# pythoncrazy/jimm

Measured on NVIDIA H100. Metric: images/sec, higher is better.
Workload: dtype f16

## Files before the change

### jimm_b200/csrc/common.cuh

```cuda
#pragma once

#include <cuda.h>
#include <cuda_bf16.h>
#include <cuda_fp16.h>
#include <cuda_fp8.h>
#include <cuda_runtime.h>
#include <stdint.h>

#include <atomic>
#include <mutex>
#include <string>

namespace jimm {

void set_last_error(const char* fmt, ...);

#define JIMM_CUDA_CHECK(expr)                                                                   \
  do {                                                                                          \
    cudaError_t _e = (expr);                                                                    \
    if (_e != cudaSuccess) {                                                                    \
      ::jimm::set_last_error("%s:%d: %s -> %s", __FILE__, __LINE__, #expr, cudaGetErrorString(_e)); \
      return -2;                                                                                \
    }                                                                                           \
  } while (0)
// ... 80 lines not shown
      : "=r"(pred));
  return pred != 0;
}

__device__ __forceinline__ void mbar_init(uint64_t* bar, uint32_t count) {
  asm volatile("mbarrier.init.shared::cta.b64 [%0], %1;" ::"r"(smem_u32(bar)), "r"(count));
}
__device__ __forceinline__ void fence_barrier_init() {
  asm volatile("fence.mbarrier_init.release.cluster;" ::: "memory");
}
__device__ __forceinline__ void fence_proxy_async_smem() {
  asm volatile("fence.proxy.async.shared::cta;" ::: "memory");
}
__device__ __forceinline__ void mbar_arrive(uint64_t* bar) {
  asm volatile("mbarrier.arrive.shared::cta.b64 _, [%0];" ::"r"(smem_u32(bar)) : "memory");
}
__device__ __forceinline__ void mbar_arrive_expect_tx(uint64_t* bar, uint32_t bytes) {
  asm volatile("mbarrier.arrive.expect_tx.shared::cta.b64 _, [%0], %1;" ::"r"(smem_u32(bar)), "r"(bytes) : "memory");
}
__device__ __forceinline__ void mbar_wait(uint64_t* bar, uint32_t parity) {
  asm volatile(
      "{\n\t.reg .pred P1;\n\t"
      "WAIT_LOOP:\n\t"
      "mbarrier.try_wait.parity.shared::cta.b64 P1, [%0], %1;\n\t"
      "@P1 bra DONE;\n\t"
      "bra WAIT_LOOP;\n\t"
      "DONE:\n\t}" ::"r"(smem_u32(bar)),
      "r"(parity)
      : "memory");
}

__device__ __forceinline__ bool mbar_test_wait(uint64_t* bar, uint32_t parity) {
  uint32_t ok;
  asm volatile(
      "{\n\t.reg .pred P1;\n\t"
      "mbarrier.test_wait.parity.shared::cta.b64 P1, [%1], %2;\n\t"
      "selp.u32 %0, 1, 0, P1;\n\t}"
      : "=r"(ok)
      : "r"(smem_u32(bar)), "r"(parity)
      : "memory");
  return ok != 0;
}

__device__ __forceinline__ void tma_prefetch_desc(const CUtensorMap* m) {
  asm volatile("prefetch.tensormap [%0];" ::"l"(reinterpret_cast<uint64_t>(m)) : "memory");
}
__device__ __forceinline__ void tma_load_2d(void* smem_dst, const CUtensorMap* m, uint64_t* bar, int c0, int c1) {
  asm volatile(
      "cp.async.bulk.tensor.2d.shared::cluster.global.mbarrier::complete_tx::bytes [%0], [%1, {%3, %4}], [%2];" ::"r"(
          smem_u32(smem_dst)),
      "l"(reinterpret_cast<uint64_t>(m)), "r"(smem_u32(bar)), "r"(c0), "r"(c1)
      : "memory");
}

__device__ __forceinline__ void tma_store_2d(const CUtensorMap* m, uint32_t smem_src, int c0, int c1) {
  asm volatile("cp.async.bulk.tensor.2d.global.shared::cta.bulk_group [%0, {%2, %3}], [%1];" ::"l"(reinterpret_cast<uint64_t>(m)),
               "r"(smem_src), "r"(c0), "r"(c1)
               : "memory");
}
__device__ __forceinline__ void tma_reduce_add_2d(const CUtensorMap* m, uint32_t smem_src, int c0, int c1) {
  asm volatile("cp.reduce.async.bulk.tensor.2d.global.shared::cta.add.tile.bulk_group [%0, {%2, %3}], [%1];" ::"l"(
                   reinterpret_cast<uint64_t>(m)),
               "r"(smem_src), "r"(c0), "r"(c1)
               : "memory");
}
__device__ __forceinline__ void tma_store_3d(const CUtensorMap* m, uint32_t smem_src, int c0, int c1, int c2) {
  asm volatile("cp.async.bulk.tensor.3d.global.shared::cta.bulk_group [%0, {%2, %3, %4}], [%1];" ::"l"(reinterpret_cast<uint64_t>(m)),
               "r"(smem_src), "r"(c0), "r"(c1), "r"(c2)
               : "memory");
}
__device__ __forceinline__ void tma_reduce_add_3d(const CUtensorMap* m, uint32_t smem_src, int c0, int c1, int c2) {
  asm volatile("cp.reduce.async.bulk.tensor.3d.global.shared::cta.add.tile.bulk_group [%0, {%2, %3, %4}], [%1];" ::"l"(
                   reinterpret_cast<uint64_t>(m)),
               "r"(smem_src), "r"(c0), "r"(c1), "r"(c2)
               : "memory");
}
__device__ __forceinline__ void tma_store_commit() { asm volatile("cp.async.bulk.commit_group;" ::: "memory"); }
__device__ __forceinline__ void tma_store_wait_read() { asm volatile("cp.async.bulk.wait_group.read 0;" ::: "memory"); }
__device__ __forceinline__ void tma_store_wait_read1() { asm volatile("cp.async.bulk.wait_group.read 1;" ::: "memory"); }
__device__ __forceinline__ void tma_store_wait_all() { asm volatile("cp.async.bulk.wait_group 0;" ::: "memory"); }

__device__ __forceinline__ uint32_t cluster_ctarank() {
  uint32_t r;
  asm volatile("mov.u32 %0, %%cluster_ctarank;" : "=r"(r));
  return r;
}
__device__ __forceinline__ void cluster_sync_all() {
  asm volatile("barrier.cluster.arrive.release.aligned;\n\tbarrier.cluster.wait.acquire.aligned;" ::: "memory");
}
__device__ __forceinline__ uint32_t mapa_shared(uint32_t local_smem_addr, uint32_t rank) {
  uint32_t r;
  asm volatile("mapa.shared::cluster.u32 %0, %1, %2;" : "=r"(r) : "r"(local_smem_addr), "r"(rank));
  return r;
}
__device__ __forceinline__ void mbar_arrive_cluster(uint32_t cluster_addr) {
  asm volatile("mbarrier.arrive.release.cluster.shared::cluster.b64 _, [%0];" ::"r"(cluster_addr) : "memory");
}
__device__ __forceinline__ uint64_t make_wgmma_desc_sw128(uint32_t smem_addr) {
  uint64_t d = 0;
  d |= static_cast<uint64_t>((smem_addr & 0x3FFFFu) >> 4);
  d |= static_cast<uint64_t>(1) << 16;
  d |= static_cast<uint64_t>(1024 >> 4) << 32;
  d |= static_cast<uint64_t>(1) << 62;
  return d;
}
template <int SW>
__device__ __forceinline__ uint64_t make_wgmma_desc(uint32_t smem_addr, uint32_t lbo) {
  static_assert(SW == 128 || SW == 64 || SW == 32, "swizzle width");
  constexpr uint64_t layout = SW == 128 ? 1 : SW == 64 ? 2 : 3;
  uint64_t d = 0;
  d |= static_cast<uint64_t>((smem_addr & 0x3FFFFu) >> 4);
  d |= static_cast<uint64_t>((lbo >> 4) & 0x3FFFu) << 16;
  d |= static_cast<uint64_t>(8 * SW >> 4) << 32;
  d |= layout << 62;
  return d;
}
__device__ __forceinline__ void wgmma_fence() { asm volatile("wgmma.fence.sync.aligned;" ::: "memory"); }
__device__ __forceinline__ void wgmma_commit() { asm volatile("wgmma.commit_group.sync.aligned;" ::: "memory"); }
template <int N>
__device__ __forceinline__ void wgmma_wait() { asm volatile("wgmma.wait_group.sync.aligned %0;" ::"n"(N) : "memory"); }
template <int R>
__device__ __forceinline__ void wgmma_fence_operands(float (&d)[R]) {
#pragma unroll
  for (int i = 0; i < R; ++i) asm volatile("" : "+f"(d[i])::"memory");
}

#define JIMM_WGMMA_D128                                                                                                                    \
  "{%0, %1, %2, %3, %4, %5, %6, %7, %8, %9, %10, %11, %12, %13, %14, %15, %16, %17, %18, %19, %20, %21, %22, %23, %24, %25, %26, %27, "     \
  "%28, %29, %30, %31, %32, %33, %34, %35, %36, %37, %38, %39, %40, %41, %42, %43, %44, %45, %46, %47, %48, %49, %50, %51, %52, %53, %54, " \
  "%55, %56, %57, %58, %59, %60, %61, %62, %63, %64, %65, %66, %67, %68, %69, %70, %71, %72, %73, %74, %75, %76, %77, %78, %79, %80, %81, " \
  "%82, %83, %84, %85, %86, %87, %88, %89, %90, %91, %92, %93, %94, %95, %96, %97, %98, %99, %100, %101, %102, %103, %104, %105, %106, "   \
  "%107, %108, %109, %110, %111, %112, %113, %114, %115, %116, %117, %118, %119, %120, %121, %122, %123, %124, %125, %126, %127}"
#define JIMM_WGMMA_D8(i) "+f"(d[i]), "+f"(d[i + 1]), "+f"(d[i + 2]), "+f"(d[i + 3]), "+f"(d[i + 4]), "+f"(d[i + 5]), "+f"(d[i + 6]), "+f"(d[i + 7])
#define JIMM_WGMMA_D128_OPERANDS                                                                                                 \
  JIMM_WGMMA_D8(0), JIMM_WGMMA_D8(8), JIMM_WGMMA_D8(16), JIMM_WGMMA_D8(24), JIMM_WGMMA_D8(32), JIMM_WGMMA_D8(40), JIMM_WGMMA_D8(48), \
      JIMM_WGMMA_D8(56), JIMM_WGMMA_D8(64), JIMM_WGMMA_D8(72), JIMM_WGMMA_D8(80), JIMM_WGMMA_D8(88), JIMM_WGMMA_D8(96),             \
      JIMM_WGMMA_D8(104), JIMM_WGMMA_D8(112), JIMM_WGMMA_D8(120)
template <int KIND>
__device__ __forceinline__ void wgmma_m64n256_ss(float (&d)[128], uint64_t adesc, uint64_t bdesc, uint32_t accumulate) {
  if constexpr (KIND == 0) {
    asm volatile("{\n\t.reg .pred p;\n\tsetp.ne.b32 p, %130, 0;\n\t"
                 "wgmma.mma_async.sync.aligned.m64n256k16.f32.f16.f16 " JIMM_WGMMA_D128 ", %128, %129, p, 1, 1, 0, 0;\n\t}"
                 : JIMM_WGMMA_D128_OPERANDS
                 : "l"(adesc), "l"(bdesc), "r"(accumulate));
  } else if constexpr (KIND == 1) {
    asm volatile("{\n\t.reg .pred p;\n\tsetp.ne.b32 p, %130, 0;\n\t"
                 "wgmma.mma_async.sync.aligned.m64n256k16.f32.bf16.bf16 " JIMM_WGMMA_D128 ", %128, %129, p, 1, 1, 0, 0;\n\t}"
                 : JIMM_WGMMA_D128_OPERANDS
                 : "l"(adesc), "l"(bdesc), "r"(accumulate));
// ... 260 lines not shown
```

### jimm_b200/csrc/gemm.cu

```cuda
#include "gemm.cuh"

#include <stdarg.h>
#include <stdio.h>
#include <stdlib.h>
#include <string.h>

#include <type_traits>

#include "common.cuh"

namespace jimm {

static constexpr int BM = GEMM_TILE_M;
static constexpr int BN = GEMM_TILE_N;
static_assert(BM == 128 && BN == 256, "the warp roles and the wgmma shape below are written for 128 x 256 tiles");
static constexpr int STAGES = 4;
static constexpr int A_STAGE_BYTES = BM * 128;
static constexpr int B_STAGE_BYTES = BN * 128;
static constexpr int STAGE_BYTES = A_STAGE_BYTES + B_STAGE_BYTES;
static constexpr int EPI_WARPS = 8;
static constexpr int EPI_BOX_ROWS = 16;
static constexpr int EPI_BUF_BYTES = EPI_BOX_ROWS * 128;
static constexpr int EPI_BUFS = 2;
static constexpr int EPI_STAGE_BYTES = EPI_WARPS * EPI_BUFS * EPI_BUF_BYTES;
// ... 288 lines not shown
    float sa = 1.f;
    if constexpr (SCALED) sa = __ldg(epi.a_scale + row);
#pragma unroll
    for (int j = 0; j < NC / 8; ++j) {
#pragma unroll
      for (int q = 0; q < 2; ++q) {
        const int col = n_tile0 + 8 * j + 2 * t + q;
        if (col < epi.N) {
          float v = acc[4 * j + 2 * h + q];
          if constexpr (SCALED) v *= sa * __ldg(epi.b_scale + col);
          if (epi.bias) v += __ldg(epi.bias + col);
          v = apply_act(v, epi.act);
          if (epi.rowadd) v += __ldg(epi.rowadd + static_cast<size_t>(add_row) * epi.N + col);
          if (epi.residual) v += epi.residual[static_cast<size_t>(out_row) * epi.ldr + col];
          store1(epi, out_row, col, v);
        }
      }
    }
  }
}


template <typename T, int OUT, int ACT>
__global__ void __launch_bounds__(NUM_THREADS, 1)
gemm_wgmma_kernel(const __grid_constant__ CUtensorMap map_a, const __grid_constant__ CUtensorMap map_b,
                  const __grid_constant__ CUtensorMap map_c, const EpiDev epi, int K) {
  constexpr bool SCALED = kScaled<T>;
  constexpr int BK = 128 / sizeof(T);
  constexpr int UK = 32 / sizeof(T);
  constexpr int TM = tile_rows(Traits<T>::DTYPE);
  constexpr int STAGE_TX = TM * 128 + B_STAGE_BYTES;
  constexpr int WG_DM = SCALED ? 0 : 64;
  constexpr int WG_DN = SCALED ? 128 : 0;
  constexpr int NC = BN - WG_DN;
  constexpr bool FUSE_LN = OUT == OUT_F32_ADD && ACT == ACT_FUSE_LN;
  constexpr int EPI_ACT = ACT == ACT_FUSE_LN ? static_cast<int>(ACT_NONE) : ACT;
  constexpr int PRODUCER_REGS = FUSE_LN ? 152 : 40;
  constexpr int CONSUMER_REGS = FUSE_LN ? 176 : 232;
  static_assert(128 * PRODUCER_REGS + 256 * CONSUMER_REGS <= NUM_THREADS * KERNEL_REGS, "register split exceeds the CTA's allocation");

  extern __shared__ uint8_t smem_raw[];
  uint8_t* smem = reinterpret_cast<uint8_t*>((reinterpret_cast<uintptr_t>(smem_raw) + 1023) & ~static_cast<uintptr_t>(1023));
  uint8_t* smem_a = smem;
  uint8_t* smem_b = smem + STAGES * A_STAGE_BYTES;
  uint8_t* epi_stage = smem + STAGES * STAGE_BYTES;
  LnQueue* lnq = reinterpret_cast<LnQueue*>(epi_stage + EPI_STAGE_BYTES);
  uint64_t* full_bar = reinterpret_cast<uint64_t*>(lnq + 1);
  uint64_t* empty_bar = full_bar + STAGES;

  const int warp_idx = threadIdx.x >> 5;
  const int lane = threadIdx.x & 31;
  const int M = epi.M, N = epi.N;
  const int m_tiles = (M + TM - 1) / TM, n_tiles = (N + BN - 1) / BN;
  const int num_tiles = m_tiles * n_tiles;
  const int num_kb = (K + BK - 1) / BK;

  pdl_launch_dependents();
  if (warp_idx == 0 && lane == 0) {
    tma_prefetch_desc(&map_a);
    tma_prefetch_desc(&map_b);
    if constexpr (OUT != OUT_GENERIC) tma_prefetch_desc(&map_c);
    for (int s = 0; s < STAGES; ++s) {
      mbar_init(&full_bar[s], 1);
      mbar_init(&empty_bar[s], EPI_WARPS);
    }
    fence_barrier_init();
  }
  if constexpr (FUSE_LN) {
    if (warp_idx == 1) {
      for (int i = lane; i < LNQ; i += 32) lnq->slot[i] = -1;
      if (lane == 0) lnq->head = lnq->tail = lnq->done = 0;
    }
  }
  __syncthreads();
  pdl_wait();

  if (warp_idx < 4) {
    setmaxnreg<KERNEL_REGS, PRODUCER_REGS>();
    if (warp_idx == 0) {
      if (lane == 0) {
        int stage = 0;
        uint32_t phase = 0;
        for (int tile = blockIdx.x; tile < num_tiles; tile += gridDim.x) {
          const int tv = epi.reverse ? num_tiles - 1 - tile : tile;
          const int m_blk = tv / n_tiles, n_blk = tv - m_blk * n_tiles;
          for (int kb = 0; kb < num_kb; ++kb) {
            mbar_wait(&empty_bar[stage], phase ^ 1);
            mbar_arrive_expect_tx(&full_bar[stage], STAGE_TX);
            tma_load_2d(smem_a + stage * A_STAGE_BYTES, &map_a, &full_bar[stage], kb * BK, m_blk * TM);
            tma_load_2d(smem_b + stage * B_STAGE_BYTES, &map_b, &full_bar[stage], kb * BK, n_blk * BN);
            if (++stage == STAGES) { stage = 0; phase ^= 1; }
          }
        }
      }
    } else if constexpr (FUSE_LN) {
      ln_worker<T>(epi, lnq, lane);
    }
  } else {
    setmaxnreg<KERNEL_REGS, CONSUMER_REGS>();
    const int wg = (warp_idx - 4) >> 2;
    const int wq = warp_idx & 3;
    uint8_t* tbuf0 = epi_stage + (warp_idx - 4) * EPI_BUFS * EPI_BUF_BYTES;
    int stage = 0;
    uint32_t phase = 0, box_count = 0;
    int ln_rg = -1, ln_cols = 0;
    float acc[NC / 2];
    for (int tile = blockIdx.x; tile < num_tiles; tile += gridDim.x) {
      const int tv = epi.reverse ? num_tiles - 1 - tile : tile;
      const int m_blk = tv / n_tiles, n_blk = tv - m_blk * n_tiles;
      int prev = -1;
      if constexpr (SCALED) {
#pragma unroll
        for (int i = 0; i < NC / 2; ++i) acc[i] = 0.f;
      }
      for (int kb = 0; kb < num_kb; ++kb) {
        mbar_wait(&full_bar[stage], phase);
        const uint64_t adesc = make_wgmma_desc_sw128(smem_u32(smem_a + stage * A_STAGE_BYTES + wg * WG_DM * 128));
        const uint64_t bdesc = make_wgmma_desc_sw128(smem_u32(smem_b + stage * B_STAGE_BYTES + wg * WG_DN * 128));
        if constexpr (SCALED) {
          float slab[NC / 2];
          wgmma_fence_operands(slab);
          wgmma_fence();
#pragma unroll
          for (int k = 0; k < BK / UK; ++k)
            wgmma_m64n128k32_e4m3_ss(slab, adesc + static_cast<uint64_t>(2 * k), bdesc + static_cast<uint64_t>(2 * k), k != 0 ? 1u : 0u);
          wgmma_commit();
          wgmma_wait<0>();
          wgmma_fence_operands(slab);
          if (lane == 0) mbar_arrive(&empty_bar[stage]);
#pragma unroll
          for (int i = 0; i < NC / 2; ++i) acc[i] += slab[i];
        } else {
          wgmma_fence_operands(acc);
          wgmma_fence();
#pragma unroll
          for (int k = 0; k < BK / UK; ++k)
            wgmma_m64n256_ss<Traits<T>::KIND>(acc, adesc + static_cast<uint64_t>(2 * k), bdesc + static_cast<uint64_t>(2 * k), (kb | k) != 0 ? 1u : 0u);
          wgmma_commit();
          wgmma_fence_operands(acc);
          if (prev >= 0) {
            wgmma_wait<1>();
            if (lane == 0) mbar_arrive(&empty_bar[prev]);
          }
          prev = stage;
        }
        if (++stage == STAGES) { stage = 0; phase ^= 1; }
      }
      if constexpr (!SCALED) {
        wgmma_wait<0>();
        wgmma_fence_operands(acc);
        if (lane == 0) mbar_arrive(&empty_bar[prev]);
      }

      const int row_base = m_blk * TM + wg * WG_DM + wq * 16;
      const int n_tile0 = n_blk * BN + wg * WG_DN;
      if constexpr (OUT == OUT_GENERIC) {
        epilogue_generic<SCALED, NC>(epi, acc, lane, row_base, n_tile0);
      } else {
        if (row_base < M && (WG_DN == 0 || n_tile0 < N))
          epilogue_tma<OUT, EPI_ACT, SCALED, NC>(&map_c, epi, acc, tbuf0, lane, row_base, n_tile0, box_count);
        if constexpr (FUSE_LN) {
          if (lane == 0 && ln_rg >= 0) ln_publish(epi, lnq, ln_rg, ln_cols);
          ln_rg = (row_base & ~31) < M ? row_base >> 5 : -1;
          ln_cols = min(BN, N - n_tile0);
        }
      }
    }
    if constexpr (FUSE_LN) {
      if (lane == 0) {
        if (ln_rg >= 0) ln_publish(epi, lnq, ln_rg, ln_cols);
        __threadfence_block();
        atomicAdd(&lnq->done, 1);
      }
    }
    if constexpr (OUT != OUT_GENERIC) {
      if (lane == 0) tma_store_wait_all();
    }
  }
}

template <typename T>
__global__ void gemm_simt_kernel(const T* __restrict__ A, int lda, const T* __restrict__ B, int ldb, int K, EpiDev epi) {
  __shared__ float As[16][17], Bs[16][17];
  const int tx = threadIdx.x, ty = threadIdx.y;
  const int row = blockIdx.y * 16 + ty, col = blockIdx.x * 16 + tx;
  float acc = 0.f;
  for (int k0 = 0; k0 < K; k0 += 16) {
    const int ar = blockIdx.y * 16 + ty, ak = k0 + tx;
    As[ty][tx] = (ar < epi.M && ak < K) ? to_float(A[static_cast<size_t>(ar) * lda + ak]) : 0.f;
    const int br = blockIdx.x * 16 + ty, bk = k0 + tx;
    Bs[ty][tx] = (br < epi.N && bk < K) ? to_float(B[static_cast<size_t>(br) * ldb + bk]) : 0.f;
    __syncthreads();
#pragma unroll
    for (int k = 0; k < 16; ++k) acc += As[ty][k] * Bs[tx][k];
    __syncthreads();
  }
  if (row < epi.M && col < epi.N) {
    int out_row, add_row;
    remap_row(epi, row, out_row, add_row);
    float v = acc;
    if constexpr (kScaled<T>) v *= epi.a_scale[row] * epi.b_scale[col];
    if (epi.bias) v += epi.bias[col];
    v = apply_act(v, epi.act);
    if (epi.rowadd) v += epi.rowadd[static_cast<size_t>(add_row) * epi.N + col];
    if (epi.residual) v += epi.residual[static_cast<size_t>(out_row) * epi.ldr + col];
    store1(epi, out_row, col, v);
  }
}

static constexpr int SMEM_BYTES = STAGES * STAGE_BYTES + EPI_STAGE_BYTES + static_cast<int>(sizeof(LnQueue)) + 2 * STAGES * 8 + 1024;
static_assert(SMEM_BYTES <= 232448, "exceeds 227 KB of shared memory");
typedef CUresult (*PFN_encodeTiled)(CUtensorMap*, CUtensorMapDataType, cuuint32_t, void*, const cuuint64_t*, const cuuint64_t*,
                                    const cuuint32_t*, const cuuint32_t*, CUtensorMapInterleave, CUtensorMapSwizzle,
                                    CUtensorMapL2promotion, CUtensorMapFloatOOBfill);

static PFN_encodeTiled get_encode_fn() {
  static std::atomic<PFN_encodeTiled> fn{nullptr};
  if (PFN_encodeTiled f = fn.load(std::memory_order_acquire)) return f;
  void* p = nullptr;
  cudaDriverEntryPointQueryResult qres;
  cudaError_t e = cudaGetDriverEntryPoint("cuTensorMapEncodeTiled", &p, cudaEnableDefault, &qres);
  if (e != cudaSuccess || qres != cudaDriverEntryPointSuccess || p == nullptr) {
    set_last_error("cudaGetDriverEntryPoint(cuTensorMapEncodeTiled) failed: %s", cudaGetErrorString(e));
    return nullptr;
  }
  fn.store(reinterpret_cast<PFN_encodeTiled>(p), std::memory_order_release);
  return reinterpret_cast<PFN_encodeTiled>(p);
}

static CUtensorMapDataType tensor_map_dtype(int dtype) {
  switch (dtype) {
// ... 39 lines not shown
  if (r != CUDA_SUCCESS) { set_last_error("cuTensorMapEncodeTiled(3d) failed: CUresult %d", static_cast<int>(r)); return -3; }
  return 0;
}

int device_sm_count() {
  static std::atomic<int> sms[DeviceOnce::kMaxDevices] = {};
  int dev = 0;
  cudaGetDevice(&dev);
  if (dev < 0 || dev >= DeviceOnce::kMaxDevices) dev = 0;
  int n = sms[dev].load(std::memory_order_relaxed);
  if (n == 0) {
    cudaDeviceGetAttribute(&n, cudaDevAttrMultiProcessorCount, dev);
    const char* env = getenv("JIMM_NUM_SMS");
    if (env && atoi(env) > 0) n = atoi(env);
    sms[dev].store(n, std::memory_order_relaxed);
  }
  return n;
}

static int check_epi(const GemmEpilogue& e, int N) {
  if (e.out == nullptr) { set_last_error("gemm: null output"); return -1; }
  if (e.ldo < N) { set_last_error("gemm: ldo (%d) < N (%d)", e.ldo, N); return -1; }
  return 0;
}
static int check_e4m3_epi(const GemmEpilogue& e) {
  if (e.a_scale == nullptr || e.b_scale == nullptr) { set_last_error("gemm: e4m3 operands need row scales for A and B"); return -1; }
  if ((reinterpret_cast<uintptr_t>(e.b_scale) & 7) != 0) { set_last_error("gemm: the B scales must be 8-byte aligned"); return -1; }
  if (e.residual || e.rowadd || e.rows_in != 0 || e.tok_pad != 0 || e.ln_cnt) {
    set_last_error("gemm: e4m3 operands support bias and activation epilogues only (no residual, row-add, row remap, token scatter or "
                   "fused LayerNorm)");
    return -1;
  }
  return 0;
}
int gemm_plan_init(GemmPlan* plan, int dtype, const void* A, int lda, const void* B, int ldb, int M, int N, int K,
                   const GemmEpilogue& epi) {
  if (M <= 0 || N <= 0 || K <= 0) { set_last_error("gemm: bad shape %dx%dx%d", M, N, K); return -1; }
  if (int rc = check_epi(epi, N)) return rc;
  if (dtype == DT_E4M3) {
    if (int rc = check_e4m3_epi(epi)) return rc;
  }
  if (epi.tok_pad != 0) {
    if (epi.tok_pad < 0 || epi.tok_pad % EPI_BOX_ROWS != 0 || M % epi.tok_pad != 0 || epi.tok_off < 0 || epi.tok_S <= 0) {
      set_last_error("gemm: token scatter needs tok_pad a positive multiple of %d dividing M (tok_pad=%d M=%d tok_off=%d tok_S=%d)", EPI_BOX_ROWS,
                     epi.tok_pad, M, epi.tok_off, epi.tok_S);
      return -1;
    }
    if (epi.residual != epi.out || epi.ldr != epi.ldo || epi.out_type != DT_F32) {
      set_last_error("gemm: token scatter reduce-adds into an fp32 output that is also the residual");
      return -1;
    }
  }
  if (int rc = make_tensor_map_2d(&plan->map_a, dtype, A, M, K, lda, tile_rows(dtype))) return rc;
  if (int rc = make_tensor_map_2d(&plan->map_b, dtype, B, N, K, ldb, BN)) return rc;
  plan->M = M; plan->N = N; plan->K = K; plan->dtype = dtype; plan->epi = epi;
  memset(&plan->map_c, 0, sizeof(plan->map_c));
  if (plan->epi.mode == 2) {
    const size_t es = dtype_size(epi.out_type);
    const bool ok = epi.rowadd == nullptr && epi.rows_in == 0 && (static_cast<size_t>(N) * es) % 16 == 0 &&
                    (epi.residual == nullptr || (epi.residual == epi.out && epi.ldr == epi.ldo && epi.out_type == DT_F32)) &&
                    (static_cast<size_t>(epi.ldo) * es) % 16 == 0 && (reinterpret_cast<uintptr_t>(epi.out) & 15) == 0 &&
                    (epi.bias == nullptr || ((reinterpret_cast<uintptr_t>(epi.bias) & 15) == 0 && N % 4 == 0)) &&
                    !(epi.residual && epi.act != ACT_NONE);
    if (ok && epi.tok_pad > 0) {
      if (int rc = make_tensor_map_3d(&plan->map_c, DT_F32, epi.out, M / epi.tok_pad, epi.tok_S, N, epi.ldo)) return rc;
    } else if (ok) {
      if (int rc = make_tensor_map_2d(&plan->map_c, epi.out_type, epi.out, M, N, epi.ldo, EPI_BOX_ROWS)) return rc;
    } else {
      plan->epi.mode = 0;
    }
  }
  if (epi.tok_pad > 0 && plan->epi.mode != 2) {
    set_last_error("gemm: the token scatter needs the TMA epilogue (mode 2, no activation, 16-byte aligned output / bias, N %% 4 == 0)");
    return -1;
  }
  return 0;
}

static EpiDev to_dev(const GemmEpilogue& e, int M, int N) {
  EpiDev d;
  d.bias = e.bias; d.rowadd = e.rowadd; d.residual = e.residual; d.out = e.out;
  d.act = e.act; d.ldr = e.ldr; d.out_type = e.out_type; d.ldo = e.ldo;
  d.rows_in = e.rows_in; d.rows_out = e.rows_out; d.row_off = e.row_off; d.mode = e.mode;
  d.M = M; d.N = N;
  d.tok_pad = e.tok_pad; d.tok_off = e.tok_off;
  d.reverse = e.reverse;
  d.ln_scale = e.ln_scale; d.ln_bias = e.ln_bias; d.ln_out = e.ln_out; d.ln_cnt = e.ln_cnt;
  d.ln_out_type = e.ln_out_type; d.ln_ldo = e.ln_ldo; d.ln_eps = e.ln_eps;
  d.a_scale = e.a_scale; d.b_scale = e.b_scale;
  return d;
}

template <typename T, int OUT, int ACT>
static int launch_one(const GemmPlan* p, int M, cudaStream_t stream) {
  auto* kernel = gemm_wgmma_kernel<T, OUT, ACT>;
  constexpr int TM = tile_rows(Traits<T>::DTYPE);
  static DeviceOnce attr_set;
  if (int rc = attr_set.run([&]() -> int {
        JIMM_CUDA_CHECK(cudaFuncSetAttribute(kernel, cudaFuncAttributeMaxDynamicSharedMemorySize, SMEM_BYTES));
        cudaFuncAttributes fa;
        JIMM_CUDA_CHECK(cudaFuncGetAttributes(&fa, kernel));
        if (fa.numRegs != KERNEL_REGS) {
          set_last_error("gemm: kernel compiled with %d registers per thread, the warpgroup register split assumes %d", fa.numRegs, KERNEL_REGS);
          return -2;
        }
        return 0;
      }))
    return rc;
  const int tiles = ((M + TM - 1) / TM) * ((p->N + BN - 1) / BN);
  const int grid = tiles < device_sm_count() ? tiles : device_sm_count();
  JIMM_CUDA_CHECK(launch_k(kernel, dim3(grid), dim3(NUM_THREADS), SMEM_BYTES, stream, 1, true, p->map_a, p->map_b, p->map_c,
                           to_dev(p->epi, M, p->N), p->K));
  note_launch();
  return 0;
}

template <typename T, int OUT>
static int launch_act(const GemmPlan* p, int M, cudaStream_t stream) {
  switch (p->epi.act) {
    case ACT_GELU_TANH: return launch_one<T, OUT, ACT_GELU_TANH>(p, M, stream);
    case ACT_QUICK_GELU: return launch_one<T, OUT, ACT_QUICK_GELU>(p, M, stream);
    default: return launch_one<T, OUT, ACT_NONE>(p, M, stream);
  }
}

template <typename T>
static int launch_tc(const GemmPlan* p, int M, cudaStream_t stream) {
  const GemmEpilogue& e = p->epi;
  if (e.mode != 2) return launch_one<T, OUT_GENERIC, ACT_NONE>(p, M, stream);
  if constexpr (!kScaled<T>) {
    if (e.residual) return gemm_fuses_ln(p, M) ? launch_one<T, OUT_F32_ADD, ACT_FUSE_LN>(p, M, stream) : launch_one<T, OUT_F32_ADD, ACT_NONE>(p, M, stream);
  }
  switch (e.out_type) {
    case DT_F16: return launch_act<T, OUT_H16>(p, M, stream);
    case DT_BF16: return launch_act<T, OUT_BF16>(p, M, stream);
    case DT_TF32: return launch_act<T, OUT_TF32>(p, M, stream);
    default: return launch_act<T, OUT_F32>(p, M, stream);
  }
}

int gemm_fuses_ln(const GemmPlan* p, int ) {
  const int nv = p->N >> 7;
  const bool width_ok = p->N % 128 == 0 && (nv <= 4 || nv == 6 || nv == 8 || nv == 9);
  const int want = p->dtype == DT_F16 ? DT_F16 : p->dtype == DT_BF16 ? DT_BF16 : DT_TF32;
  return p->epi.ln_cnt != nullptr && p->epi.ln_out_type == want && width_ok && p->epi.mode == 2 && p->epi.residual != nullptr && p->epi.tok_pad == 0;
}

int gemm_plan_run(const GemmPlan* p0, int M_override, cudaStream_t stream, int reverse) {
  const int M = (M_override > 0 && M_override <= p0->M) ? M_override : p0->M;
  if (p0->epi.tok_pad > 0 && M % p0->epi.tok_pad != 0) {
    set_last_error("gemm: token scatter runs whole samples (M=%d, tok_pad=%d)", M, p0->epi.tok_pad);
    return -1;
  }
  GemmPlan local;
  const GemmPlan* p = p0;
  if (reverse != p0->epi.reverse) { local = *p0; local.epi.reverse = reverse; p = &local; }
  switch (p->dtype) {
    case DT_F16: return launch_tc<__half>(p, M, stream);
    case DT_BF16: return launch_tc<__nv_bfloat16>(p, M, stream);
    case DT_F32:
    case DT_TF32: return launch_tc<float>(p, M, stream);
    case DT_E4M3: return launch_tc<__nv_fp8_e4m3>(p, M, stream);
  }
  set_last_error("gemm: bad dtype %d", p->dtype);
  return -1;
// ... 20 lines not shown
```

### jimm_b200/csrc/gemm.cuh

```cuda
#pragma once
#include <cuda.h>
#include <cuda_runtime.h>
#include <stdint.h>

namespace jimm {

enum DType : int { DT_F32 = 0, DT_F16 = 1, DT_BF16 = 2, DT_TF32 = 3, DT_E4M3 = 4 };
enum Act : int { ACT_NONE = 0, ACT_GELU_TANH = 1, ACT_QUICK_GELU = 2 };

inline size_t dtype_size(int dt) { return (dt == DT_F32 || dt == DT_TF32) ? 4 : dt == DT_E4M3 ? 1 : 2; }

constexpr int GEMM_TILE_M = 128;
constexpr int GEMM_TILE_N = 256;

struct GemmEpilogue {
  const float* bias = nullptr;
  int act = ACT_NONE;
  const float* rowadd = nullptr;
  const float* residual = nullptr;
  int ldr = 0;
  void* out = nullptr;
  int out_type = DT_F32;
  int ldo = 0;
  int tok_pad = 0, tok_off = 0, tok_S = 0;
  int reverse = 0;
  int rows_in = 0, rows_out = 0, row_off = 0;
  int mode = 2;
  const float* ln_scale = nullptr;
  const float* ln_bias = nullptr;
  void* ln_out = nullptr;
  int ln_out_type = DT_F16, ln_ldo = 0;
  float ln_eps = 1e-6f;
  int* ln_cnt = nullptr;
  const float* a_scale = nullptr;
  const float* b_scale = nullptr;
};

struct GemmPlan {
  CUtensorMap map_a, map_b, map_c;
  int M = 0, N = 0, K = 0;
  int dtype = DT_F16;
  GemmEpilogue epi;
};

int gemm_plan_init(GemmPlan* plan, int dtype, const void* A, int lda, const void* B, int ldb, int M, int N, int K,
                   const GemmEpilogue& epi);
int gemm_plan_run(const GemmPlan* plan, int M_override, cudaStream_t stream, int reverse = 0);

int gemm_simt_run(int dtype, const void* A, int lda, const void* B, int ldb, int M, int N, int K, const GemmEpilogue& epi,
                  cudaStream_t stream);

int gemm_fuses_ln(const GemmPlan* plan, int M_override);

int device_sm_count();

}
```

### jimm_b200/csrc/model.cu

```cuda
#include <stdarg.h>
#include <stdio.h>
#include <stdlib.h>
#include <string.h>

#include <algorithm>
#include <atomic>
#include <cmath>
#include <map>
#include <tuple>
#include <memory>
#include <utility>
#include <string>
#include <vector>

#include "../../include/jimm_b200.h"
#include "comm.cuh"
#include "common.cuh"
#include "gemm.cuh"
#include "kernels.cuh"

namespace jimm {

static thread_local char g_err[1024] = "";
void set_last_error(const char* fmt, ...) {
// ... 1445 lines not shown
int jimm_encoder_forward(jimm_model_t* m, const float* x, int B, int S, float* out, void* stream) {
  JIMM_TRY(check_sub(m, JIMM_ENCODER, B, S, x, out));
  cudaStream_t s = static_cast<cudaStream_t>(stream);
  const size_t row = static_cast<size_t>(S) * m->vis.D;
  return for_chunks(B, m->max_batch, [&](int b0, int nb) {
    JIMM_CUDA_CHECK(cudaMemcpyAsync(m->ws.enc.x, x + b0 * row, nb * row * sizeof(float), cudaMemcpyDeviceToDevice, s));
    JIMM_TRY(run_encoder(m, &m->vis.enc, nb, S, s, m->ws.enc));
    JIMM_CUDA_CHECK(cudaMemcpyAsync(out + b0 * row, m->ws.enc.x, nb * row * sizeof(float), cudaMemcpyDeviceToDevice, s));
    return 0;
  });
}

int jimm_map_head_forward(jimm_model_t* m, const float* x, int B, int S, float* out, void* stream) {
  JIMM_TRY(check_sub(m, JIMM_MAPHEAD, B, S, x, out));
  cudaStream_t s = static_cast<cudaStream_t>(stream);
  const size_t row = static_cast<size_t>(S) * m->vis.D;
  return for_chunks(B, m->max_batch, [&](int b0, int nb) {
    JIMM_TRY(cast_run(x + b0 * row, m->ws.enc.h, m->cdt, nb * row, s));
    return run_map_head(m, nb, S, out + static_cast<size_t>(b0) * m->vis.D, s);
  });
}

static int ensure_copy_stream(jimm_model* m) {
  if (m->copy_stream) return 0;
  JIMM_CUDA_CHECK(cudaStreamCreateWithFlags(&m->copy_stream, cudaStreamNonBlocking));
  for (int i = 0; i < jimm_model::kHostSlices; ++i) {
    JIMM_CUDA_CHECK(cudaEventCreateWithFlags(&m->ev_copied[i], cudaEventDisableTiming));
    JIMM_CUDA_CHECK(cudaEventCreateWithFlags(&m->ev_consumed[i], cudaEventDisableTiming));
  }
  JIMM_CUDA_CHECK(cudaEventCreateWithFlags(&m->ev_start, cudaEventDisableTiming));
  return 0;
}

static void host_slices(const jimm_model* m, int nb, int* sizes, size_t bytes_per_image = 0) {
  for (int i = 0; i < jimm_model::kHostSlices; ++i) sizes[i] = 0;
  sizes[0] = nb;
  if (const char* env = getenv("JIMM_HOST_SLICES")) {
    int k = 0, acc = 0;
    for (const char* q = env; *q && k < jimm_model::kHostSlices - 1;) {
      const int v = atoi(q);
      if (v <= 0 || acc + v >= nb) break;
      sizes[k++] = v;
      acc += v;
      while (*q && *q != ',') ++q;
      if (*q == ',') ++q;
    }
    sizes[k] = nb - acc;
    return;
  }
  if (nb < 128) return;
  if (bytes_per_image && static_cast<size_t>(nb) * bytes_per_image < (static_cast<size_t>(64) << 20)) return;
  static const int head_div = [] { const char* env = getenv("JIMM_HOST_HEAD_DIV"); return (env && atoi(env) > 0) ? atoi(env) : 4; }();
  const int S = m->vis.S, D = m->vis.D, Mm = m->vis.enc.c.M;
  const int sms = device_sm_count();
  auto cost = [&](int n) {
    const long mt = (static_cast<long>(n) * S + GEMM_TILE_M - 1) / GEMM_TILE_M;
    auto rounds = [&](int N) { return (mt * ((N + GEMM_TILE_N - 1) / GEMM_TILE_N) + sms - 1) / sms; };
    return static_cast<double>(D) * rounds(3 * D) + static_cast<double>(D) * rounds(D) + static_cast<double>(D) * rounds(Mm) +
           static_cast<double>(Mm) * rounds(D);
  };
  int best = nb / head_div;
  double best_cost = 1e30;
  for (int c0 = nb / head_div; c0 <= nb / 3; ++c0) {
    const double cst = cost(c0) + cost(nb - c0) + 1e-3 * c0 * D;
    if (cst < best_cost) { best_cost = cst; best = c0; }
  }
  sizes[0] = best;
  sizes[1] = nb - best;
}

static int vit_forward_host_impl(jimm_model_t* m, const void* img_host, int in_dtype, int B, float* out_host, cudaStream_t s,
                                 jimm_preproc_t* pre, int Hin, int Win) {
  JIMM_TRY(ensure_copy_stream(m));
  const size_t img_elems = static_cast<size_t>(m->vis.img) * m->vis.img * m->vis.C;
  const size_t src_bytes = pre ? static_cast<size_t>(Hin) * Win * 3 : img_elems * dtype_size(in_dtype);
  const int tower_dtype = pre ? (m->cdt == DT_TF32 ? JIMM_F32 : m->cdt) : in_dtype;
  const int od = vision_out_dim(m);
  const int kind = pre ? 1 : 0;
  if (pre) {
    const size_t need = static_cast<size_t>(m->max_batch) * src_bytes;
    if (need > m->ws.in_u8_bytes) {
      std::lock_guard<std::mutex> no_capture(g_capture_mu);
      JIMM_CUDA_CHECK(cudaDeviceSynchronize());
      if (m->ws.in_u8) cudaFree(m->ws.in_u8);
      m->ws.in_u8 = nullptr; m->ws.in_u8_bytes = 0;
      JIMM_CUDA_CHECK(cudaMalloc(&m->ws.in_u8, need));
      m->ws.in_u8_bytes = need;
      m->host_chain = false;
    }
  }
  return for_chunks(B, m->max_batch, [&](int b0, int nb) {
    int sizes[jimm_model::kHostSlices];
    host_slices(m, nb, sizes, src_bytes);
    if (pre && img_elems % 4) {
      for (int i = 0; i + 1 < jimm_model::kHostSlices && sizes[i + 1] > 0; ++i) {
        const int r = sizes[i] % 4;
        sizes[i] -= r;
        sizes[i + 1] += r;
      }
    }
    bool same_layout = m->host_chain && m->host_chain_stream == s && m->host_chain_kind == kind;
    for (int i = 0; i < jimm_model::kHostSlices; ++i) same_layout = same_layout && sizes[i] == m->host_chain_sizes[i];
    if (!same_layout) {
      JIMM_CUDA_CHECK(cudaEventRecord(m->ev_start, s));
      JIMM_CUDA_CHECK(cudaStreamWaitEvent(m->copy_stream, m->ev_start, 0));
      for (int i = 0; i < jimm_model::kHostSlices; ++i) {
        if (m->slot_recorded[i]) JIMM_CUDA_CHECK(cudaStreamWaitEvent(m->copy_stream, m->ev_consumed[i], 0));
        m->slot_recorded[i] = false;
        m->host_chain_sizes[i] = sizes[i];
      }
// ... 156 lines not shown
```

### jimm_b200/csrc/probe.cu

```cuda
#include "../../include/jimm_b200.h"
#include "common.cuh"
#include "gemm.cuh"

namespace jimm {

int make_tensor_map_2d(CUtensorMap* map, int dtype, const void* ptr, int rows, int cols, int ld, int box_rows);

namespace {

constexpr int PB_STAGES = 12;
constexpr int PB_STAGE_BYTES = 128 * 128;

__device__ __forceinline__ void tma_load_2d_multicast(void* smem_dst, const CUtensorMap* m, uint64_t* bar, int c0, int c1, uint16_t mask) {
  asm volatile(
      "cp.async.bulk.tensor.2d.shared::cluster.global.mbarrier::complete_tx::bytes.multicast::cluster [%0], [%1, {%3, %4}], [%2], %5;" ::"r"(
          smem_u32(smem_dst)),
      "l"(reinterpret_cast<uint64_t>(m)), "r"(smem_u32(bar)), "r"(c0), "r"(c1), "h"(mask)
      : "memory");
}

template <int CS>
__global__ void __launch_bounds__(64, 1) l2_probe_kernel(const __grid_constant__ CUtensorMap map_full, const __grid_constant__ CUtensorMap map_part,
                                                         int mode, int iters, int total_rows) {
  extern __shared__ uint8_t smem_raw[];
  uint8_t* smem = reinterpret_cast<uint8_t*>((reinterpret_cast<uintptr_t>(smem_raw) + 1023) & ~static_cast<uintptr_t>(1023));
  uint64_t* full = reinterpret_cast<uint64_t*>(smem + PB_STAGES * PB_STAGE_BYTES);
  uint64_t* empty = full + PB_STAGES;
  const uint32_t rank = CS > 1 ? cluster_ctarank() : 0;
  const int cluster_id = blockIdx.x / CS;
  const bool shared_writes = CS > 1 && mode == 2;
  if (threadIdx.x == 0) {
    for (int i = 0; i < PB_STAGES; ++i) {
      mbar_init(&full[i], 1);
      mbar_init(&empty[i], shared_writes ? CS : 1);
    }
    fence_barrier_init();
  }
  __syncthreads();
  if (CS > 1) cluster_sync_all();
  const int tiles = total_rows / 128;
  if (threadIdx.x == 0) {
    int st = 0;
    uint32_t ph = 0;
    for (int it = 0; it < iters; ++it) {
      const long long tile = mode == 0 ? (static_cast<long long>(blockIdx.x) * iters + it) : (static_cast<long long>(cluster_id) * iters + it);
      const int row = static_cast<int>((tile * 7919) % tiles) * 128;
      mbar_wait(&empty[st], ph ^ 1);
      mbar_arrive_expect_tx(&full[st], PB_STAGE_BYTES);
      if (mode == 2 && CS > 1) {
        constexpr int part = 128 / CS;
        tma_load_2d_multicast(smem + st * PB_STAGE_BYTES + rank * part * 128, &map_part, &full[st], 0, row + rank * part,
                              static_cast<uint16_t>((1u << CS) - 1));
      } else {
        tma_load_2d(smem + st * PB_STAGE_BYTES, &map_full, &full[st], 0, row);
      }
      if (++st == PB_STAGES) { st = 0; ph ^= 1; }
    }
  } else if (threadIdx.x == 32) {
    int st = 0;
    uint32_t ph = 0;
    for (int it = 0; it < iters; ++it) {
      mbar_wait(&full[st], ph);
      if (shared_writes) {
        for (uint32_t r = 0; r < CS; ++r)
          asm volatile("mbarrier.arrive.relaxed.cluster.shared::cluster.b64 _, [%0];" ::"r"(mapa_shared(smem_u32(&empty[st]), r)) : "memory");
      } else {
        mbar_arrive(&empty[st]);
      }
      if (++st == PB_STAGES) { st = 0; ph ^= 1; }
    }
  }
  __syncthreads();
// ... 48 lines not shown
```

Baseline: 11930.

## Run GEMM as 2-CTA clusters multicasting the shared B tile

The persistent wgmma GEMM now launches 2-CTA clusters. Each CTA in a pair handles an adjacent M tile and the two share one N tile. Each CTA TMA-multicasts half of the B tile to both CTAs, so B traffic from L2 per CTA is halved. Stage release now needs arrivals from both CTAs' consumer warps via cross-CTA mbarrier arrives. This adds cluster syncs and couples the two CTAs' pipelines, and it changes the grid sizing and the host cost model to count tile pairs.

Measured after the change: 12010 (median of 6 runs). No clear change (+0.6%).

```diff
diff --git a/jimm_b200/csrc/common.cuh b/jimm_b200/csrc/common.cuh
--- a/jimm_b200/csrc/common.cuh
+++ b/jimm_b200/csrc/common.cuh
@@ -156,6 +156,13 @@
       "l"(reinterpret_cast<uint64_t>(m)), "r"(smem_u32(bar)), "r"(c0), "r"(c1)
       : "memory");
 }
+__device__ __forceinline__ void tma_load_2d_multicast(void* smem_dst, const CUtensorMap* m, uint64_t* bar, int c0, int c1, uint16_t mask) {
+  asm volatile(
+      "cp.async.bulk.tensor.2d.shared::cluster.global.mbarrier::complete_tx::bytes.multicast::cluster [%0], [%1, {%3, %4}], [%2], %5;" ::"r"(
+          smem_u32(smem_dst)),
+      "l"(reinterpret_cast<uint64_t>(m)), "r"(smem_u32(bar)), "r"(c0), "r"(c1), "h"(mask)
+      : "memory");
+}
 
 __device__ __forceinline__ void tma_store_2d(const CUtensorMap* m, uint32_t smem_src, int c0, int c1) {
   asm volatile("cp.async.bulk.tensor.2d.global.shared::cta.bulk_group [%0, {%2, %3}], [%1];" ::"l"(reinterpret_cast<uint64_t>(m)),
@@ -198,7 +205,7 @@
   return r;
 }
 __device__ __forceinline__ void mbar_arrive_cluster(uint32_t cluster_addr) {
-  asm volatile("mbarrier.arrive.release.cluster.shared::cluster.b64 _, [%0];" ::"r"(cluster_addr) : "memory");
+  asm volatile("mbarrier.arrive.shared::cluster.b64 _, [%0];" ::"r"(cluster_addr) : "memory");
 }
 __device__ __forceinline__ uint64_t make_wgmma_desc_sw128(uint32_t smem_addr) {
   uint64_t d = 0;
diff --git a/jimm_b200/csrc/gemm.cu b/jimm_b200/csrc/gemm.cu
--- a/jimm_b200/csrc/gemm.cu
+++ b/jimm_b200/csrc/gemm.cu
@@ -364,8 +364,9 @@
   const int lane = threadIdx.x & 31;
   const int M = epi.M, N = epi.N;
   const int m_tiles = (M + TM - 1) / TM, n_tiles = (N + BN - 1) / BN;
-  const int num_tiles = m_tiles * n_tiles;
+  const int num_pairs = ((m_tiles + 1) >> 1) * n_tiles;
   const int num_kb = (K + BK - 1) / BK;
+  const uint32_t rank = cluster_ctarank(), peer = rank ^ 1u;
 
   pdl_launch_dependents();
   if (warp_idx == 0 && lane == 0) {
@@ -374,7 +375,7 @@
     if constexpr (OUT != OUT_GENERIC) tma_prefetch_desc(&map_c);
     for (int s = 0; s < STAGES; ++s) {
       mbar_init(&full_bar[s], 1);
-      mbar_init(&empty_bar[s], EPI_WARPS);
+      mbar_init(&empty_bar[s], 2 * EPI_WARPS);
     }
     fence_barrier_init();
   }
@@ -384,7 +385,7 @@
       if (lane == 0) lnq->head = lnq->tail = lnq->done = 0;
     }
   }
-  __syncthreads();
+  cluster_sync_all();
   pdl_wait();
 
   if (warp_idx < 4) {
@@ -393,14 +394,20 @@
       if (lane == 0) {
         int stage = 0;
         uint32_t phase = 0;
-        for (int tile = blockIdx.x; tile < num_tiles; tile += gridDim.x) {
-          const int tv = epi.reverse ? num_tiles - 1 - tile : tile;
-          const int m_blk = tv / n_tiles, n_blk = tv - m_blk * n_tiles;
+        for (int pair = blockIdx.x >> 1; pair < num_pairs; pair += gridDim.x >> 1) {
+          const int pv = epi.reverse ? num_pairs - 1 - pair : pair;
+          const int m_pair = pv / n_tiles, n_blk = pv - m_pair * n_tiles;
+          const int m_blk = 2 * m_pair + static_cast<int>(rank);
+          const bool a_live = m_blk * TM < M;
+          const bool b_hi_live = n_blk * BN + BN / 2 < N;
+          const uint32_t tx = STAGE_TX - (a_live ? 0 : TM * 128) - (b_hi_live ? 0 : B_STAGE_BYTES / 2);
           for (int kb = 0; kb < num_kb; ++kb) {
             mbar_wait(&empty_bar[stage], phase ^ 1);
-            mbar_arrive_expect_tx(&full_bar[stage], STAGE_TX);
-            tma_load_2d(smem_a + stage * A_STAGE_BYTES, &map_a, &full_bar[stage], kb * BK, m_blk * TM);
-            tma_load_2d(smem_b + stage * B_STAGE_BYTES, &map_b, &full_bar[stage], kb * BK, n_blk * BN);
+            mbar_arrive_expect_tx(&full_bar[stage], tx);
+            if (a_live) tma_load_2d(smem_a + stage * A_STAGE_BYTES, &map_a, &full_bar[stage], kb * BK, m_blk * TM);
+            if (rank == 0 || b_hi_live)
+              tma_load_2d_multicast(smem_b + stage * B_STAGE_BYTES + rank * (BN / 2) * 128, &map_b, &full_bar[stage], kb * BK,
+                                    n_blk * BN + static_cast<int>(rank) * (BN / 2), 0x3);
             if (++stage == STAGES) { stage = 0; phase ^= 1; }
           }
         }
@@ -417,9 +424,14 @@
     uint32_t phase = 0, box_count = 0;
     int ln_rg = -1, ln_cols = 0;
     float acc[NC / 2];
-    for (int tile = blockIdx.x; tile < num_tiles; tile += gridDim.x) {
-      const int tv = epi.reverse ? num_tiles - 1 - tile : tile;
-      const int m_blk = tv / n_tiles, n_blk = tv - m_blk * n_tiles;
+    auto release = [&](int s) {
+      mbar_arrive(&empty_bar[s]);
+      mbar_arrive_cluster(mapa_shared(smem_u32(&empty_bar[s]), peer));
+    };
+    for (int pair = blockIdx.x >> 1; pair < num_pairs; pair += gridDim.x >> 1) {
+      const int pv = epi.reverse ? num_pairs - 1 - pair : pair;
+      const int m_pair = pv / n_tiles, n_blk = pv - m_pair * n_tiles;
+      const int m_blk = 2 * m_pair + static_cast<int>(rank);
       int prev = -1;
       if constexpr (SCALED) {
 #pragma unroll
@@ -439,7 +451,7 @@
           wgmma_commit();
           wgmma_wait<0>();
           wgmma_fence_operands(slab);
-          if (lane == 0) mbar_arrive(&empty_bar[stage]);
+          if (lane == 0) release(stage);
 #pragma unroll
           for (int i = 0; i < NC / 2; ++i) acc[i] += slab[i];
         } else {
@@ -452,7 +464,7 @@
           wgmma_fence_operands(acc);
           if (prev >= 0) {
             wgmma_wait<1>();
-            if (lane == 0) mbar_arrive(&empty_bar[prev]);
+            if (lane == 0) release(prev);
           }
           prev = stage;
         }
@@ -461,7 +473,7 @@
       if constexpr (!SCALED) {
         wgmma_wait<0>();
         wgmma_fence_operands(acc);
-        if (lane == 0) mbar_arrive(&empty_bar[prev]);
+        if (lane == 0) release(prev);
       }
 
       const int row_base = m_blk * TM + wg * WG_DM + wq * 16;
@@ -489,6 +501,8 @@
       if (lane == 0) tma_store_wait_all();
     }
   }
+  __syncwarp();
+  cluster_sync_all();
 }
 
 template <typename T>
@@ -634,7 +648,7 @@
     }
   }
   if (int rc = make_tensor_map_2d(&plan->map_a, dtype, A, M, K, lda, tile_rows(dtype))) return rc;
-  if (int rc = make_tensor_map_2d(&plan->map_b, dtype, B, N, K, ldb, BN)) return rc;
+  if (int rc = make_tensor_map_2d(&plan->map_b, dtype, B, N, K, ldb, BN / 2)) return rc;
   plan->M = M; plan->N = N; plan->K = K; plan->dtype = dtype; plan->epi = epi;
   memset(&plan->map_c, 0, sizeof(plan->map_c));
   if (plan->epi.mode == 2) {
@@ -674,10 +688,10 @@
 }
 
 template <typename T, int OUT, int ACT>
-static int launch_one(const GemmPlan* p, int M, cudaStream_t stream) {
+static int pair_slots() {
   auto* kernel = gemm_wgmma_kernel<T, OUT, ACT>;
-  constexpr int TM = tile_rows(Traits<T>::DTYPE);
   static DeviceOnce attr_set;
+  static int clusters[DeviceOnce::kMaxDevices];
   if (int rc = attr_set.run([&]() -> int {
         JIMM_CUDA_CHECK(cudaFuncSetAttribute(kernel, cudaFuncAttributeMaxDynamicSharedMemorySize, SMEM_BYTES));
         cudaFuncAttributes fa;
@@ -686,13 +700,47 @@
           set_last_error("gemm: kernel compiled with %d registers per thread, the warpgroup register split assumes %d", fa.numRegs, KERNEL_REGS);
           return -2;
         }
+        cudaLaunchConfig_t cfg = {};
+        cudaLaunchAttribute attr;
+        attr.id = cudaLaunchAttributeClusterDimension;
+        attr.val.clusterDim.x = 2;
+        attr.val.clusterDim.y = 1;
+        attr.val.clusterDim.z = 1;
+        cfg.gridDim = dim3(2);
+        cfg.blockDim = dim3(NUM_THREADS);
+        cfg.dynamicSmemBytes = SMEM_BYTES;
+        cfg.attrs = &attr;
+        cfg.numAttrs = 1;
+        int n = 0;
+        JIMM_CUDA_CHECK(cudaOccupancyMaxActiveClusters(&n, kernel, &cfg));
+        if (n < 1) {
+          set_last_error("gemm: no 2-CTA cluster of the GEMM kernel fits on this device");
+          return -2;
+        }
+        int dev = 0;
+        cudaGetDevice(&dev);
+        clusters[dev < 0 || dev >= DeviceOnce::kMaxDevices ? 0 : dev] = n;
         return 0;
       }))
     return rc;
-  const int tiles = ((M + TM - 1) / TM) * ((p->N + BN - 1) / BN);
-  const int grid = tiles < device_sm_count() ? tiles : device_sm_count();
-  JIMM_CUDA_CHECK(launch_k(kernel, dim3(grid), dim3(NUM_THREADS), SMEM_BYTES, stream, 1, true, p->map_a, p->map_b, p->map_c,
-                           to_dev(p->epi, M, p->N), p->K));
+  int dev = 0;
+  cudaGetDevice(&dev);
+  const int n = clusters[dev < 0 || dev >= DeviceOnce::kMaxDevices ? 0 : dev];
+  const int cap = device_sm_count() / 2;
+  return cap < 1 ? 1 : n < cap ? n : cap;
+}
+
+int gemm_pair_slots() { return pair_slots<__half, OUT_H16, ACT_NONE>(); }
+
+template <typename T, int OUT, int ACT>
+static int launch_one(const GemmPlan* p, int M, cudaStream_t stream) {
+  constexpr int TM = tile_rows(Traits<T>::DTYPE);
+  const int slots = pair_slots<T, OUT, ACT>();
+  if (slots < 0) return slots;
+  const int pairs = ((M + 2 * TM - 1) / (2 * TM)) * ((p->N + BN - 1) / BN);
+  const int grid = 2 * (pairs < slots ? pairs : slots);
+  JIMM_CUDA_CHECK(launch_k(gemm_wgmma_kernel<T, OUT, ACT>, dim3(grid), dim3(NUM_THREADS), SMEM_BYTES, stream, 2, true, p->map_a, p->map_b,
+                           p->map_c, to_dev(p->epi, M, p->N), p->K));
   note_launch();
   return 0;
 }
diff --git a/jimm_b200/csrc/gemm.cuh b/jimm_b200/csrc/gemm.cuh
--- a/jimm_b200/csrc/gemm.cuh
+++ b/jimm_b200/csrc/gemm.cuh
@@ -53,5 +53,6 @@
 int gemm_fuses_ln(const GemmPlan* plan, int M_override);
 
 int device_sm_count();
+int gemm_pair_slots();
 
 }
diff --git a/jimm_b200/csrc/model.cu b/jimm_b200/csrc/model.cu
--- a/jimm_b200/csrc/model.cu
+++ b/jimm_b200/csrc/model.cu
@@ -1521,10 +1521,10 @@
   if (bytes_per_image && static_cast<size_t>(nb) * bytes_per_image < (static_cast<size_t>(64) << 20)) return;
   static const int head_div = [] { const char* env = getenv("JIMM_HOST_HEAD_DIV"); return (env && atoi(env) > 0) ? atoi(env) : 4; }();
   const int S = m->vis.S, D = m->vis.D, Mm = m->vis.enc.c.M;
-  const int sms = device_sm_count();
+  const int slots = std::max(1, gemm_pair_slots());
   auto cost = [&](int n) {
-    const long mt = (static_cast<long>(n) * S + GEMM_TILE_M - 1) / GEMM_TILE_M;
-    auto rounds = [&](int N) { return (mt * ((N + GEMM_TILE_N - 1) / GEMM_TILE_N) + sms - 1) / sms; };
+    const long mp = (static_cast<long>(n) * S + 2 * GEMM_TILE_M - 1) / (2 * GEMM_TILE_M);
+    auto rounds = [&](int N) { return (mp * ((N + GEMM_TILE_N - 1) / GEMM_TILE_N) + slots - 1) / slots; };
     return static_cast<double>(D) * rounds(3 * D) + static_cast<double>(D) * rounds(D) + static_cast<double>(D) * rounds(Mm) +
            static_cast<double>(Mm) * rounds(D);
   };
diff --git a/jimm_b200/csrc/probe.cu b/jimm_b200/csrc/probe.cu
--- a/jimm_b200/csrc/probe.cu
+++ b/jimm_b200/csrc/probe.cu
@@ -10,14 +10,6 @@
 
 constexpr int PB_STAGES = 12;
 constexpr int PB_STAGE_BYTES = 128 * 128;
-
-__device__ __forceinline__ void tma_load_2d_multicast(void* smem_dst, const CUtensorMap* m, uint64_t* bar, int c0, int c1, uint16_t mask) {
-  asm volatile(
-      "cp.async.bulk.tensor.2d.shared::cluster.global.mbarrier::complete_tx::bytes.multicast::cluster [%0], [%1, {%3, %4}], [%2], %5;" ::"r"(
-          smem_u32(smem_dst)),
-      "l"(reinterpret_cast<uint64_t>(m)), "r"(smem_u32(bar)), "r"(c0), "r"(c1), "h"(mask)
-      : "memory");
-}
 
 template <int CS>
 __global__ void __launch_bounds__(64, 1) l2_probe_kernel(const __grid_constant__ CUtensorMap map_full, const __grid_constant__ CUtensorMap map_part,
```
